# Gabriel-SGama/Semantic-SuperPoint

Hardware: AMD Instinct MI355X
Metric: image-pairs/sec at 240x320 bs32 (pair training step) (higher is better)
Workload: dtype f32

## Files before the change

include/ssp_hip.h:

```cpp
#ifndef SSP_HIP_H
#define SSP_HIP_H

#include <stddef.h>
#include <stdint.h>

#ifdef __cplusplus
extern "C" {
#endif

typedef struct ssp_handle ssp_handle;

enum { SSP_ARCH_GAUSS2 = 0, SSP_ARCH_GAUSS2_SSMALL = 1 };
enum { SSP_NREP = 32 };

typedef struct {
  int arch;
  int n_classes;
  int max_batch;
  int height;
  int width;
  int n_match;
  int n_non;
  int dense_loss;
} ssp_config;
// ... 98 lines not shown
                      void* workspace_dev, size_t workspace_bytes, void* stream);

int ssp_op_conv_bf16(const void* in_dev, const float* w_oihw_dev, const float* bias_dev, void* out_dev, int n, int h, int w,
                     int cin, int cout, int ksize, int in_mode, const float* in_scale_dev, const float* in_shift_dev,
                     double* stats_dev, int transpose_flip, int in_f32, int out_f32, void* pool_out_dev,
                     const float* pool_gamma_dev, void* workspace_dev, size_t workspace_bytes, void* stream);

int ssp_op_conv_wgrad_bf16(const void* x_dev, const void* dy_dev, float* dw_oihw_dev, int n, int h, int w, int cin, int cout,
                           int ksize, int in_mode, const float* in_scale_dev, const float* in_shift_dev, int dy_f32,
                           void* workspace_dev, size_t workspace_bytes, void* stream);

int ssp_op_bn_bwd_bf16(const void* y_dev, const void* dout_dev, const float* gamma_dev, const float* stats4_dev, void* dy_dev,
                       float* dgamma_dev, float* dbeta_dev, float* dbias_dev, double* sums_dev, int n, int h, int w, int c, int cs,
                       int relu, int pool, void* stream);

int ssp_op_labels(const float* labels2d_dev, const float* mask2d_dev, float* target_dev, float* cellmask_dev, int b,
                  int h, int w, void* stream);

int ssp_op_detector_loss(const float* semi_nhwc_dev, int cs, const float* labels2d_dev, const float* mask2d_dev, int b, int h,
                         int w, void* scratch_dev, size_t scratch_bytes, float* loss_dev, float* dsemi_nhwc_dev, void* stream);

int ssp_op_sem_loss(const float* sout_nhwc_dev, int cs, const int64_t* labels_dev, int b, int h, int w, int n_classes, int algo,
                    void* scratch_dev, size_t scratch_bytes, float* loss_dev, float* dsout_nhwc_dev, void* stream);

int ssp_op_sem_predict(const float* sout_nhwc_dev, int cs, const int64_t* labels_dev, int b, int h, int w, int n_classes,
                       uint8_t* pred_dev, int64_t* confusion_dev, void* stream);
int ssp_sem_predict(ssp_handle* h, int slot, const int64_t* labels_dev, uint8_t* pred_dev, int64_t* confusion_dev, void* stream);

int ssp_op_warp_image(const float* img_dev, const float* inv_h_dev, float* out_dev, int b, int h, int w, int nearest,
                      void* stream);
// ... 276 lines not shown
```

semantic-superpoint_amd/csrc/bn_kernels.hip.h:

```cpp
#pragma once
#include <hip/hip_runtime.h>
#include <stdint.h>

#include "conv_mfma.hip.h"

namespace sspk {

template <typename T>
__device__ __forceinline__ float4 ld4(const T* p) {
  if constexpr (sizeof(T) == 4) {
    return *reinterpret_cast<const float4*>(p);
  } else {
    const u32x2 v = *reinterpret_cast<const u32x2*>(p);
    return make_float4(bf16_lo(v[0]), bf16_hi(v[0]), bf16_lo(v[1]), bf16_hi(v[1]));
  }
}
template <typename T>
__device__ __forceinline__ void st4(T* p, float4 v) {
  if constexpr (sizeof(T) == 4) {
    *reinterpret_cast<float4*>(p) = v;
  } else {
    u32x2 o;
    o[0] = pack_bf16(v.x, v.y);
    o[1] = pack_bf16(v.z, v.w);
// ... 639 lines not shown
#pragma unroll
    for (int t = 0; t < 9; ++t) red[tid * 10 + t] = wacc[i >> 1][t][i & 1];
    __syncthreads();
    if (tid < 160) {
      const int qq = tid / 10, t = tid - qq * 10;
      if (t < 9) {
        float sum = 0.f;
#pragma unroll
        for (int r = 0; r < 16; ++r) sum += red[(r * 16 + qq) * 10 + t];
        facc_add(dw + (qq * 4 + i) * 9 + t, sum);
      }
    }
  }
}

template <typename T = float>
__device__ __forceinline__ void bn_bwd_sums_body(const BnBwdArgs& a0, const BnBwdArgs& a1, int nviews, float* __restrict__ dgamma,
                                                 float* __restrict__ dbeta) {
  const int t = blockIdx.x * blockDim.x + threadIdx.x;
  if ((t >> 5) >= ((a0.C + 7) & ~7)) return;
  const int c = min(t >> 5, a0.C - 1), r = t & 31;
  const bool writer = r == 0 && (t >> 5) < a0.C;
  for (int v = 0; v < nviews; ++v) {
    const BnBwdArgs& a = v ? a1 : a0;
    const int C = a.C;
    double s1, s2;
    replica_sums(a.sums, C, c, r, s1, s2);
    if (a.pool_fix && a.gamma[c] == 0.f) {
      double part = 0.0;
      if (a.beta[c] > 0.f) {
// ... 197 lines not shown
```

semantic-superpoint_amd/csrc/ssp.hip:

```cpp
#include "../../include/ssp_hip.h"

#include <hip/hip_runtime.h>

#include <cmath>
#include <cstdarg>
#include <cstdio>
#include <cstdlib>
#include <algorithm>
#include <cstring>
#include <string>
#include <vector>

#include "bn_kernels.hip.h"
#include "conv_mfma.hip.h"
#include "conv1x1_group.hip.h"
#include "conv_wino.hip.h"
#include "conv_wino_pipe.hip.h"
#include "conv_wino_p2.hip.h"
#include "conv_wino4.hip.h"
#include "wgrad_wino4.hip.h"
#include "wgrad_wino_fused.hip.h"
#include "conv_bf16.hip.h"
#include "conv_bf16_ws.hip.h"
#include "wgrad_bf16.hip.h"
// ... 136 lines not shown
  float *wpk_fwd, *wpk_bwd, *wpk_heads_bwd;
  float* partial;
  size_t partial_floats;
  size_t partial_used = 0;
  struct WredBQueue* rq_bf16 = nullptr;
  WredJobs rjobs{};
  bool bsums_fused[16] = {};
  bool sums_lazy[16] = {};
  bool fin_pending[16] = {};
  double fin_count[16] = {};
  bool apply_fused[16] = {};
  bool bf16_fuse_apply = true;
  StepAccum* accum;
  float* dots;
  bool desc_gather = true;
  int32_t *csr_off = nullptr, *csr_match = nullptr;
  float* csr_weight = nullptr;
  float* g_rows = nullptr;
  float* dense_coef;
  int sout_cs;
  int conv_algo;
  bool pk_w4_fwd[16] = {}, pk_w4_bwd[16] = {};
  float *wpk_g1_fwd[16] = {}, *wpk_g1_bwd[16] = {};
  bool pk_g1[16] = {};
  float* g1_partial = nullptr;
  TailJobs tail = {};
  int g1_partial_slabs = 0;
  int packed_algo = -1;
  bool packed_bwd = false;
  struct GraphEntry { std::vector<unsigned char> key; hipGraphExec_t exec; };
// ... 915 lines not shown
  const BnBwdArgs& a1 = a[nviews - 1];
  const int nq = (a0.C + 3) / 4, rows = 256 / nq;
  const long npix = (long)a0.N * (POOL ? a0.H / 2 : a0.H) * (POOL ? a0.W / 2 : a0.W);
  int nb = cdiv(npix, rows);
  if (nb > 1024) nb = 1024;
  if (!sums_done)
    hipLaunchKernelGGL((bn_bwd_kernel<RELU, POOL, false, T>), dim3(nb, nviews), dim3(256), 0, st, a0, a1, a0, a1);
  hipLaunchKernelGGL(bn_bwd_sums_kernel<T>, dim3(cdiv(a0.C * 32, 256)), dim3(256), 0, st, a0, a1, nviews, dgamma, dbeta);
  if (!skip_apply)
    hipLaunchKernelGGL((bn_bwd_kernel<RELU, POOL, true, T>), dim3(nb, nviews), dim3(256), 0, st, a0, a1, a0, a1);
  HIPCHK(hipGetLastError());
  return 0;
}

template <typename K>
static int l0_resident_grid(K kern, const ssp_handle* h, int nviews, long rows, int W) {
  static int per_cu = 0, per_cu_w = 0;
  if (per_cu_w != W) { per_cu = 0; per_cu_w = W; }
  if (per_cu == 0 && (hipOccupancyMaxActiveBlocksPerMultiprocessor(&per_cu, kern, 256, l0_lds_bytes(W)) != hipSuccess || per_cu < 1)) {
    (void)hipGetLastError();
    per_cu = -1;
  }
  if (per_cu < 1) return l0_grid(rows);
  const long g = std::max(1L, (long)per_cu * (h ? h->n_cu : 256) / std::max(1, nviews));
  return (int)std::min(rows, g);
}

#include "bf16_host.hip.h"

static int flush_wgrad_reduce_bf16(ssp_handle* h, hipStream_t st) { return h->rq_bf16 != nullptr ? h->rq_bf16->flush(st) : 0; }

static int ensure_aux_stream(ssp_handle* h);
static bool desc_gather_env();

struct DetHostRegion { float* lo; size_t n; long long* shadow; const ssp_handle* owner; };
static std::vector<DetHostRegion> g_det_regions;
static int g_det_mode = -1;
static int g_det_device = -1;
static bool det_mode() {
  if (g_det_mode < 0) { const char* e = getenv("SSP_DETERMINISTIC"); g_det_mode = (e != nullptr && atoi(e) != 0) ? 1 : 0; }
  return g_det_mode == 1;
}
static int det_upload() {
  DetRegion tab[DET_MAX_REGIONS];
  int n = 0;
  for (const DetHostRegion& r : g_det_regions) {
    if (n == DET_MAX_REGIONS) return fail(-3, "deterministic mode: more than %d fp32 scatter targets are bound in this process", DET_MAX_REGIONS);
    tab[n].lo = r.lo; tab[n].hi = r.lo + r.n; tab[n].shadow = r.shadow; ++n;
// ... 109 lines not shown
int ssp_create(const ssp_config* cfg, ssp_handle** out) {
  if (!cfg || !out) return fail(-1, "null argument");
  if (cfg->arch != SSP_ARCH_GAUSS2 && cfg->arch != SSP_ARCH_GAUSS2_SSMALL) return fail(-1, "unknown arch %d", cfg->arch);
  if (cfg->height % 8 || cfg->width % 8 || cfg->height <= 0 || cfg->width <= 0)
    return fail(-1, "height/width must be positive multiples of 8 (got %dx%d)", cfg->height, cfg->width);
  if (cfg->width > L0_MAX_W) return fail(-1, "width must be <= %d (row images of the first-layer kernels)", L0_MAX_W);
  if (cfg->max_batch < 1 || cfg->max_batch > 1024) return fail(-1, "max_batch must be in 1..1024");
  if (cfg->arch == SSP_ARCH_GAUSS2_SSMALL && cfg->n_classes > 192) return fail(-1, "n_classes must be <= 192");
  ssp_handle* h = new ssp_handle();
  h->cfg = *cfg;
  if (h->cfg.n_classes <= 0) h->cfg.n_classes = 133;
  if (h->cfg.n_match <= 0) h->cfg.n_match = 1000;
  if (h->cfg.n_non <= 0) h->cfg.n_non = 100;
  h->conv_algo = g_default_conv_algo;
  h->desc_gather = desc_gather_env();
  h->rq_bf16 = new WredBQueue();
  AlgoScope algo(h);
  build_layers(h);
  h->bound = false;
  h->n_cu = device_cu_count();
  h->ws_bytes = carve(h, nullptr);
  h->prof_family = 0; h->ev_used = 0; h->prof_flops = h->prof_bytes = h->prof_exec_flops = 0; h->prof_launches = 0;
  *out = h;
  return 0;
}

void ssp_destroy(ssp_handle* h) {
  if (!h) return;
  det_release(h);
  delete h->rq_bf16;
// ... 481 lines not shown
  if (pack_forked) {
    CHK(ensure_aux_stream(h));
    CHK(pack_fork.fork(st, h->aux_stream, h->ev_pack_fork, h->ev_pack_join));
    CHK(pack_all(h, for_backward, SS.n, N, H, W, h->aux_stream));
  } else {
    CHK(pack_all(h, for_backward, SS.n, N, H, W, st));
  }
  {
    const LayerDesc& d = h->L[0];
    Slot &S0 = *SS.s[0], &S1 = *SS.s[SS.n - 1];
    if (bf16_path())
      hipLaunchKernelGGL(conv0_direct_kernel<uint16_t>, dim3(l0_resident_grid(conv0_direct_kernel<uint16_t>, h, SS.n, (long)N * H, W), SS.n), dim3(256), l0_lds_bytes(W), st, S0.x, S1.x, P(h, d.w_off),
                         P(h, d.b_off), reinterpret_cast<uint16_t*>(S0.Y[0]), reinterpret_cast<uint16_t*>(S1.Y[0]),
                         train ? S0.bn[0].stats : nullptr, train ? S1.bn[0].stats : nullptr, N, H, W);
    else
    hipLaunchKernelGGL(conv0_direct_kernel<float>, dim3(l0_resident_grid(conv0_direct_kernel<float>, h, SS.n, (long)N * H, W), SS.n), dim3(256), l0_lds_bytes(W), st, S0.x, S1.x, P(h, d.w_off),
                       P(h, d.b_off), S0.Y[0], S1.Y[0], train ? S0.bn[0].stats : nullptr, train ? S1.bn[0].stats : nullptr,
                       N, H, W);
    HIPCHK(hipGetLastError());
    if (train && bn_lazy_env() && !bf16_path()) { h->fin_pending[0] = true; h->fin_count[0] = (double)N * H * W; }
    else CHK(bn_finalize(h, SS.s, SS.n, 0, (double)N * H * W, train, st));
  }
  CHK(pack_fork.join());
  for (int l = 1; l < 8; ++l) {
    int lh, lw; layer_res(l, H, W, lh, lw);
    CHK(conv_layer_fwd(h, SS, l, l - 1, N, lh, lw, layer_in_mode(l), train, st));
  }
  const int Hc = H / 8, Wc = W / 8;
  auto pointwise = [&](const int* layers, int n) -> int {
    bool grouped = true;
    for (int i = 0; i < n; ++i) grouped = grouped && h->pk_g1[layers[i]];
    if (!grouped) {
      BnDeferred fin;
// ... 63 lines not shown
    v.dy_cs = dy_cs; v.dy_co = dy_co; v.count = (double)N * H * W;
    v.k12 = S.bn[l].k12;
    have_pool = have_pool && v.apool != nullptr;
  }
  const bool fused = h->bsums_fused[l];
  h->bsums_fused[l] = false;
  if (fused) h->tap_route[l] |= TAP_BSUMS_FUSED;
  h->apply_fused[l] = false;
  const bool raw_pool = pool_after && l < 8 && SS.s[0]->pool_raw[l];
  if ((fused || raw_pool) && pool_after)
    for (int k = 0; k < SS.n; ++k) a[k].pool_fix = 1;
  const BnBwdArgs &a0 = a[0], &a1 = a[SS.n - 1];
  float *dg = Gd(h, d.g_off), *db = Gd(h, d.be_off);
  if (l == 0) {
    const int nb1 = l0_resident_grid(bn_bwd_reduce_l0_kernel<float>, h, SS.n, (long)N * H, W);
    const int nb2 = l0_resident_grid(bn_bwd_apply_l0_kernel<float>, h, SS.n, (long)N * H, W);
    if (!fused)
      hipLaunchKernelGGL(bn_bwd_reduce_l0_kernel<float>, dim3(nb1, SS.n), dim3(256), l0_lds_bytes(W), st, a0, a1, P(h, d.w_off), P(h, d.b_off));
    hipLaunchKernelGGL(bn_bwd_sums_kernel<float>, dim3(cdiv(64 * 32, 256)), dim3(256), 0, st, a0, a1, SS.n, dg, db);
    hipLaunchKernelGGL(bn_bwd_apply_l0_kernel<float>, dim3(nb2, SS.n), dim3(256), l0_lds_bytes(W), st, a0, a1, P(h, d.w_off), P(h, d.b_off),
                       Gd(h, d.w_off));
    h->tap_route[0] |= TAP_WG_L0 << TAP_WG_SHIFT;
  } else if (relu && pool_after && have_pool && d.cout % 4 == 0 && d_cs == d.cout && d_co == 0) {
    const long npix = (long)N * (H / 2) * (W / 2);
    const int rows = 256 / (d.cout / 4);
    const int nb = std::max(1, std::min(cdiv(npix, rows), 1024));
    if (!fused && !SS.s[0]->pool_raw[l]) hipLaunchKernelGGL(bn_bwd_reduce_pool_kernel, dim3(nb, SS.n), dim3(256), 0, st, a0, a1, P(h, d.be_off));
    else if (!fused) {
      BnBwdArgs r[2] = {a[0], a[SS.n - 1]};
      for (int k = 0; k < 2; ++k) {
        r[k].y = r[k].apool; r[k].y_cs = d.cout; r[k].y_co = 0; r[k].H = H / 2; r[k].W = W / 2;
      }
      hipLaunchKernelGGL((bn_bwd_kernel<true, false, false>), dim3(nb, SS.n), dim3(256), 0, st, r[0], r[1], r[0], r[1]);
    }
    hipLaunchKernelGGL(bn_bwd_sums_kernel<float>, dim3(cdiv(d.cout * 32, 256)), dim3(256), 0, st, a0, a1, SS.n, dg, db);
    const bool defer = l >= 1 && l < 8 && layer_in_mode(l) == 1 && dy_cs == d.cout && dy_co == 0 && SS.s[0]->y_cs[l] == d.cout &&
// ... 938 lines not shown
}

int ssp_pair_step_phase(ssp_handle* h, const ssp_pair_inputs* in, float* scalars_dev, int phase, void* stream) {
  return pair_step_impl(h, in, scalars_dev, phase, (hipStream_t)stream);
}

size_t ssp_grad_early_offset(const ssp_handle* h) { return h ? h->L[EARLY_SPLIT_LAYER].w_off : 0; }

int ssp_pair_step_graph(ssp_handle* h, const ssp_pair_inputs* in, float* scalars_dev, int phase, int sample_indices,
                        void* stream) {
  if (!h || !h->bound) return fail(-1, "handle not bound");
  if (!in || !scalars_dev) return fail(-1, "null argument");
  hipStream_t st = (hipStream_t)stream;
  if (st == nullptr) return fail(-1, "ssp_pair_step_graph needs a non-default stream (stream capture)");
  if (h->tap_arena != nullptr) return fail(-1, "ssp_pair_step_graph: backward taps are on (ssp_debug_backward_taps); they need the eager step");
  std::vector<unsigned char> key(sizeof(ssp_pair_inputs) + sizeof(void*) + 5 * sizeof(int));
  {
    ssp_pair_inputs k;
    memcpy(&k, in, sizeof(k));
    k.seed = 0;
    memcpy(key.data(), &k, sizeof(k));
    memcpy(key.data() + sizeof(k), &scalars_dev, sizeof(void*));
    const int extra[5] = {phase, sample_indices, h->conv_algo, bf16_fuse_apply_env() ? 1 : 0,
                          h->desc_gather ? 1 : 0};
    memcpy(key.data() + sizeof(k) + sizeof(void*), extra, sizeof(extra));
  }
  hipGraphExec_t exec = nullptr;
  for (auto& g : h->graphs)
    if (g.key == key) { exec = g.exec; break; }
  if (exec == nullptr) {
    if (h->prof_family != 0) return fail(-1, "ssp_pair_step_graph: disable ssp_profile_enable before capturing");
    if (h->graphs.size() >= 16) {
      (void)hipGraphExecDestroy(h->graphs.front().exec);
      h->graphs.erase(h->graphs.begin());
    }
    hipGraph_t graph = nullptr;
    HIPCHK(hipStreamBeginCapture(st, hipStreamCaptureModeThreadLocal));
    int rc = 0;
    if (sample_indices && phase != 2) {
// ... 41 lines not shown
    if (workspace_bytes >= img) {
      hipStream_t st = (hipStream_t)stream;
      float* wpk = reinterpret_cast<float*>(workspace_dev);
      G1PackJobs G;
      G.n = 0;
      int nb = 0;
      g1_add_pack(G, nb, w_oihw_dev, wpk, transpose_flip ? cin : cout, transpose_flip ? cout : cin, transpose_flip ? 1 : 0);
      hipLaunchKernelGGL(pack_g1_kernel, dim3(nb), dim3(256), 0, st, G);
      HIPCHK(hipGetLastError());
      G1Layer y;
      y.in[0] = in_dev; y.in_cs = cin; y.in_co = 0; y.out[0] = out_dev; y.out_cs = cout; y.out_co = 0; y.wpk = wpk; y.bias = bias_dev;
      y.scale[0] = in_scale_dev; y.shift[0] = in_shift_dev; y.stats[0] = stats_dev; y.K = cin; y.N = cout;
      return launch_g1(&y, 1, 1, (long)n * hh * w, in_mode, device_cu_count(), st);
    }
  }
  const bool wino = wino_ok(ksize, cin) && in_mode != 2;
  const int nchunks = cdiv(cin, CK), ncob = cdiv(cout, NB);
  const size_t need = (size_t)ncob * nchunks * pk_taps(ksize) * CK * NB * sizeof(float);
  if (workspace_bytes < need) return fail(-4, "ssp_op_conv workspace too small (%zu < %zu)", workspace_bytes, need);
  if (bf16_path() && ksize == 3 && cin % CK == 0 && in_mode != 2)
    return fail(-3, "ssp_op_conv: conv algorithm 12 has no fp32 3x3 kernel for Cin %% 16 == 0 (use ssp_op_conv_bf16 or another algorithm)");
  hipStream_t st = (hipStream_t)stream;
  float* wpk = reinterpret_cast<float*>(workspace_dev);
  const bool w4 = wino && ksize == 3 && w4_eligible(nullptr, 1, n, hh, w, cin, cout);
  if (!transpose_flip) CHK(launch_pack(w_oihw_dev, wpk, cout, cin, ksize, 0, wino, st, w4));
  else CHK(launch_pack(w_oihw_dev, wpk, cin, cout, ksize, 1, wino, st, w4));
  ConvCall c;
  c.in = in_dev; c.in_cs = cin; c.in_co = 0; c.cin = cin; c.wpk = wpk; c.bias = bias_dev; c.out = out_dev; c.out_cs = cout;
  c.out_co = 0; c.cout = cout; c.in_scale = in_scale_dev; c.in_shift = in_shift_dev; c.stats = stats_dev; c.N = n;
  c.H = hh; c.W = w; c.ks = ksize; c.in_mode = in_mode; c.nchunks = nchunks; c.ncob = ncob; c.wino = wino;
// ... 1257 lines not shown
  HIPCHK(hipMemsetAsync(sums_dev, 0, 2 * (size_t)c * NREP * sizeof(double), st));
  BnBwdArgs a;
  a.y = y_dev; a.dout = dout_dev; a.dy = dy_dev; a.scale = stats4_dev; a.shift = stats4_dev + c; a.mean = stats4_dev + 2 * c;
  a.invstd = stats4_dev + 3 * c; a.gamma = gamma_dev; a.sums = sums_dev; a.dbias = dbias_dev; a.N = n; a.H = hh; a.W = w;
  a.C = c; a.y_cs = cs; a.y_co = 0; a.d_cs = cs; a.d_co = 0; a.dy_cs = cs; a.dy_co = 0; a.count = (double)n * hh * w;
  float* k12 = nullptr;
  HIPCHK(hipMallocAsync((void**)&k12, 2 * c * sizeof(float), st));
  a.k12 = k12; a.x = nullptr; a.apool = nullptr; a.beta = nullptr; a.pool_fix = 0;
  if (relu && pool) CHK((launch_bn_bwd<true, true>(&a, 1, dgamma_dev, dbeta_dev, st)));
  else if (relu) CHK((launch_bn_bwd<true, false>(&a, 1, dgamma_dev, dbeta_dev, st)));
  else CHK((launch_bn_bwd<false, false>(&a, 1, dgamma_dev, dbeta_dev, st)));
  HIPCHK(hipFreeAsync(k12, st));
  return 0;
}

int ssp_op_bn_bwd_bf16(const void* y_dev, const void* dout_dev, const float* gamma_dev, const float* stats4_dev, void* dy_dev,
                       float* dgamma_dev, float* dbeta_dev, float* dbias_dev, double* sums_dev, int n, int hh, int w, int c, int cs,
                       int relu, int pool, void* stream) {
  if (cs < c || (cs & 3)) return fail(-1, "ssp_op_bn_bwd_bf16: the channel stride must be a multiple of 4 and >= C");
  if (!relu) return fail(-3, "ssp_op_bn_bwd_bf16: only the ReLU layers run on bf16 tensors");
  hipStream_t st = (hipStream_t)stream;
  HIPCHK(hipMemsetAsync(sums_dev, 0, 2 * (size_t)c * NREP * sizeof(double), st));
  BnBwdArgs a;
  a.y = reinterpret_cast<const float*>(y_dev); a.dout = reinterpret_cast<const float*>(dout_dev); a.dy = reinterpret_cast<float*>(dy_dev);
  a.scale = stats4_dev; a.shift = stats4_dev + c; a.mean = stats4_dev + 2 * c;
  a.invstd = stats4_dev + 3 * c; a.gamma = gamma_dev; a.sums = sums_dev; a.dbias = dbias_dev; a.N = n; a.H = hh; a.W = w;
  a.C = c; a.y_cs = cs; a.y_co = 0; a.d_cs = cs; a.d_co = 0; a.dy_cs = cs; a.dy_co = 0; a.count = (double)n * hh * w;
  float* k12 = nullptr;
  HIPCHK(hipMallocAsync((void**)&k12, 2 * c * sizeof(float), st));
  a.k12 = k12; a.x = nullptr; a.apool = nullptr; a.beta = nullptr; a.pool_fix = 0;
// ... 295 lines not shown
```

semantic-superpoint_amd/lib.py:

```python
import ctypes as C
import math
import os
from collections import OrderedDict

import numpy as np
import torch

from . import hipbuild as _build

ARCHS = {"SuperPointNet_gauss2": 0, "SuperPointNet_gauss2_ssmall": 1}
SCALAR_NAMES = ["loss", "loss_det", "loss_det_warp", "loss_desc", "loss_sem", "loss_sem_warp", "positive_dist",
                "negative_dist", "eta_det", "eta_desc", "eta_sem"]
N_SCALARS = 16
NREP = 32
SAMPLER_MAX_MATCHES = 8192
PROF = {"none": 0, "conv3x3_fwd": 1, "conv3x3_dgrad": 2, "conv3x3_wgrad": 3, "conv_big_fwd": 4, "conv3x3_all": 5,
        "conv3x3_every": 6}
PROF_KERNELS = ["conv_wino4_kernel", "conv_wino_pipe_kernel", "conv_wino_p2_kernel", "wgrad_wino_kernel", "wgrad_wino4_kernel",
                "other", "conv_bf16_kernel", "wgrad_bf16_kernel"]


class SspConfig(C.Structure):
    _fields_ = [("arch", C.c_int), ("n_classes", C.c_int), ("max_batch", C.c_int), ("height", C.c_int),
                ("width", C.c_int), ("n_match", C.c_int), ("n_non", C.c_int), ("dense_loss", C.c_int)]
# ... 71 lines not shown
                ("nms_dist", C.c_int32), ("border_remove", C.c_int32), ("top_k", C.c_int32), ("subpixel", C.c_int32)]


_lib = None

EXPORTS = ["ssp_last_error", "ssp_create", "ssp_destroy", "ssp_param_count", "ssp_bn_channel_count",
           "ssp_bn_layer_count", "ssp_workspace_bytes", "ssp_bind", "ssp_forward", "ssp_backward", "ssp_zero_grad",
           "ssp_pair_step", "ssp_adam_step", "ssp_sample_indices", "ssp_profile_enable", "ssp_profile_read", "ssp_profile_read_executed",
           "ssp_op_conv", "ssp_op_conv_wgrad", "ssp_op_labels", "ssp_op_sparse_loss", "ssp_op_bn_bwd", "ssp_op_bn_bwd_strided",
           "ssp_debug_buffer", "ssp_debug_conv_knobs", "ssp_set_conv_algo", "ssp_op_warp_image", "ssp_op_erode", "ssp_op_warp_labels",
           "ssp_export_workspace_bytes", "ssp_export_max_points", "ssp_export_points", "ssp_op_homoadapt_views",
           "ssp_op_flatten_detection", "ssp_op_combine_heatmap", "ssp_op_heatmap_points", "ssp_op_soft_argmax_points", "ssp_detector_heatmap", "ssp_op_heatmap_nms", "ssp_op_dense_loss",
           "ssp_op_sample_homographies", "ssp_op_warp_labels_full", "ssp_op_sem_finalize", "ssp_adam_step_scaled",
           "ssp_pair_step_phase", "ssp_grad_early_offset", "ssp_pair_step_graph", "ssp_handle_set_conv_algo",
           "ssp_op_detector_loss", "ssp_debug_occupancy", "ssp_sample_indices_cell", "ssp_op_warp_labels_px",
           "ssp_op_warp_labels_full_px", "ssp_profile_read_kernel", "ssp_op_label_quantize", "ssp_profile_pause", "ssp_op_conv_bf16", "ssp_op_conv_wgrad_bf16", "ssp_op_bn_bwd_bf16", "ssp_build_id",
           "ssp_set_deterministic", "ssp_get_deterministic", "ssp_clock_probe", "ssp_op_sem_loss",
           "ssp_describe_workspace_bytes", "ssp_describe_points", "ssp_op_sample_descriptors", "ssp_match_workspace_bytes",
           "ssp_match_two_way", "ssp_debug_backward_taps", "ssp_debug_backward_tap_floats", "ssp_debug_backward_tap",
           "ssp_eval_repeatability", "ssp_eval_ransac_workspace_bytes", "ssp_eval_ransac",
           "ssp_op_photometric_draw", "ssp_op_photometric_apply",
           "ssp_shapes_workspace_bytes", "ssp_op_shapes_draw", "ssp_op_shapes_render", "ssp_op_warp_points_scatter",
           "ssp_op_sem_predict", "ssp_sem_predict",
           "ssp_track_workspace_bytes", "ssp_op_track_update", "ssp_op_track_select", "ssp_op_track_points",
           "ssp_op_point_classes", "ssp_point_classes", "ssp_filter_workspace_bytes", "ssp_op_filter_points",
           "ssp_match_two_way_classes",
           "ssp_det_eval_workspace_bytes", "ssp_op_det_tp_fp", "ssp_op_det_tp_fp_points", "ssp_det_pr_curve_workspace_bytes",
           "ssp_op_det_pr_curve", "ssp_op_sparse_loss_path",
           "ssp_eval_pixel_homographies", "ssp_eval_accumulate",
           "ssp_epi_ransac_workspace_bytes", "ssp_epi_ransac", "ssp_op_filter_matches",
           "ssp_pose_from_fundamental", "ssp_pose_chain",
# ... 108 lines not shown
        if os.environ.get("SSP_HIP_LIB") is None:
            raise
    lib.ssp_debug_buffer.argtypes = [vp, i, C.c_char_p, C.POINTER(vp), C.POINTER(C.c_size_t)]
    if hasattr(lib, "ssp_debug_backward_taps"):
        lib.ssp_debug_backward_taps.argtypes = [vp, vp, C.c_size_t, C.c_uint]
        lib.ssp_debug_backward_tap_floats.argtypes = [vp, C.c_uint]
        lib.ssp_debug_backward_tap_floats.restype = C.c_size_t
        lib.ssp_debug_backward_tap.argtypes = [vp, i, i, i, C.POINTER(C.c_size_t), C.POINTER(C.c_size_t), C.POINTER(C.c_uint)]
    lib.ssp_debug_conv_knobs.argtypes = [i, i]
    lib.ssp_debug_occupancy.argtypes = [i]
    lib.ssp_set_conv_algo.argtypes = [i]
    lib.ssp_op_warp_image.argtypes = [vp, vp, vp, i, i, i, i, vp]
    lib.ssp_op_erode.argtypes = [vp, vp, i, i, i, i, vp]
    lib.ssp_op_warp_labels.argtypes = [vp, vp, vp, i, i, i, vp]
    lib.ssp_op_bn_bwd.argtypes = [vp, vp, vp, vp, vp, vp, vp, vp, vp, i, i, i, i, i, i, vp]
    lib.ssp_op_bn_bwd_strided.argtypes = [vp, vp, vp, vp, vp, vp, vp, vp, vp, i, i, i, i, i, i, i, vp]
    lib.ssp_op_labels.argtypes = [vp, vp, vp, vp, i, i, i, vp]
    lib.ssp_op_sparse_loss.argtypes = [vp, vp, vp, vp, vp, i, i, i, i, i, i, i, C.c_float, C.c_float, vp, vp, vp, vp]
    try:
        lib.ssp_op_sparse_loss_path.argtypes = [vp, vp, vp, vp, vp, i, i, i, i, i, i, i, C.c_float, C.c_float, vp, vp, vp, i, vp, vp, vp, vp]
    except AttributeError:
        if os.environ.get("SSP_HIP_LIB") is None:
            raise
    ep = C.POINTER(SspExportParams)
    lib.ssp_export_workspace_bytes.argtypes = [ep]
    lib.ssp_export_workspace_bytes.restype = C.c_size_t
    lib.ssp_export_max_points.argtypes = [ep]
    lib.ssp_export_points.argtypes = [vp, ep, i] + [C.POINTER(vp)] * 7 + [vp]
    lib.ssp_op_homoadapt_views.argtypes = [vp, vp, vp, vp, i, i, i, vp]
    lib.ssp_op_flatten_detection.argtypes = [vp, vp, vp, i, i, i, vp]
# ... 961 lines not shown
    lib = load_library()
    _need_gpu(y_nhwc, "y")
    N, H, W, cs = y_nhwc.shape
    Cc = gamma.numel()
    dev = y_nhwc.device
    stats4 = torch.cat([scale, shift, mean, invstd]).contiguous()
    dy = torch.zeros_like(y_nhwc) if cs != Cc else torch.empty_like(y_nhwc)
    dg, db, dbias = (torch.zeros(Cc, dtype=torch.float32, device=dev) for _ in range(3))
    sums = torch.zeros(NREP * 2 * Cc, dtype=torch.float64, device=dev)
    with torch.cuda.device(dev):
        _check(lib.ssp_op_bn_bwd_strided(_ptr(y_nhwc), _ptr(dout_nhwc), _ptr(gamma), _ptr(stats4), _ptr(dy), _ptr(dg),
                                         _ptr(db), _ptr(dbias), _ptr(sums), N, H, W, Cc, cs, int(relu), int(pool), _stream()))
    return dy, dg, db, dbias


def op_bn_bwd_bf16(y_nhwc, dout_nhwc, gamma, scale, shift, mean, invstd, pool=False):
    lib = load_library()
    _need_gpu(y_nhwc, "y")
    if y_nhwc.dtype != torch.bfloat16 or dout_nhwc.dtype != torch.bfloat16:
        raise RuntimeError("y and dout must be bfloat16")
    N, H, W, cs = y_nhwc.shape
    Cc = gamma.numel()
    dev = y_nhwc.device
    stats4 = torch.cat([scale, shift, mean, invstd]).contiguous()
    dy = torch.zeros_like(y_nhwc)
    dg, db, dbias = (torch.zeros(Cc, dtype=torch.float32, device=dev) for _ in range(3))
    sums = torch.zeros(NREP * 2 * Cc, dtype=torch.float64, device=dev)
    with torch.cuda.device(dev):
        _check(lib.ssp_op_bn_bwd_bf16(_ptr(y_nhwc), _ptr(dout_nhwc), _ptr(gamma), _ptr(stats4), _ptr(dy), _ptr(dg), _ptr(db),
                                      _ptr(dbias), _ptr(sums), N, H, W, Cc, cs, 1, int(pool), _stream()))
# ... 1234 lines not shown
```

Before: 2439.

## Stream layer-0 BN-backward dout through an LDS ring with async buffer loads

Adds a layer-0 fused BN-backward/weight-gradient kernel that prefetches dout rows into a per-wave LDS ring buffer using buffer_load-to-LDS, with hand-written waitcnt and ds_read asm. Prefetches sit several slots ahead so global memory latency overlaps the recompute-and-accumulate math. It is enabled by default through an env toggle, with the old kernel kept as a fallback when LDS would exceed 64KB. It also adds a standalone l0 wgrad op, a conv0 fast path in the generic conv op, and a graph-cache key field. The extra LDS per block may lower occupancy.

```diff
diff --git a/include/ssp_hip.h b/include/ssp_hip.h
--- a/include/ssp_hip.h
+++ b/include/ssp_hip.h
@@ -136,6 +136,10 @@
                        float* dgamma_dev, float* dbeta_dev, float* dbias_dev, double* sums_dev, int n, int h, int w, int c, int cs,
                        int relu, int pool, void* stream);
 
+int ssp_op_l0_wgrad(const float* x_dev, const float* dout_dev, const float* w0_dev, const float* b0_dev, const float* gamma_dev,
+                    const float* stats4_dev, float* dw0_dev, float* dgamma_dev, float* dbeta_dev, double* sums_dev, int n, int h,
+                    int w, void* stream);
+
 int ssp_op_labels(const float* labels2d_dev, const float* mask2d_dev, float* target_dev, float* cellmask_dev, int b,
                   int h, int w, void* stream);
 
diff --git a/semantic-superpoint_amd/csrc/bn_kernels.hip.h b/semantic-superpoint_amd/csrc/bn_kernels.hip.h
--- a/semantic-superpoint_amd/csrc/bn_kernels.hip.h
+++ b/semantic-superpoint_amd/csrc/bn_kernels.hip.h
@@ -677,6 +677,134 @@
   }
 }
 
+constexpr int L0R_DP = 4;
+static inline size_t l0_ring_lds_bytes(int W) { return (size_t)4 * L0R_DP * 2048 + l0_lds_bytes(W) + 32 * sizeof(float); }
+__global__ __launch_bounds__(256) void bn_bwd_apply_l0_ring_kernel(const BnBwdArgs a0, const BnBwdArgs a1,
+                                                                   const float* __restrict__ w0, const float* __restrict__ b0,
+                                                                   float* __restrict__ dw) {
+  const BnBwdArgs& a = blockIdx.y ? a1 : a0;
+  const float* __restrict__ x = a.x;
+  extern __shared__ float l0_rows[];
+  float* const red = l0_rows;
+  float* const imgs = l0_rows + 4 * L0R_DP * 512;
+  static_assert(4 * L0R_DP * 512 >= 256 * 10, "the weight-gradient reduction runs in the ring's LDS");
+  const int tid = threadIdx.x;
+  const int q = tid & 15, pl = tid >> 4;
+  const int wave = tid >> 6, lane = tid & 63;
+  const int c0 = q * 4;
+  L0Conv cv;
+  cv.load(w0, b0, c0);
+  f32x2 sc2[2], sh2[2], is2[2], nm2[2], nk1[2], nk2[2], gs2[2];
+#pragma unroll
+  for (int h = 0; h < 2; ++h) {
+    const int c = c0 + 2 * h;
+    sc2[h] = f32x2{a.scale[c], a.scale[c + 1]}; sh2[h] = f32x2{a.shift[c], a.shift[c + 1]};
+    is2[h] = f32x2{a.invstd[c], a.invstd[c + 1]};
+    nm2[h] = f32x2{-a.mean[c] * a.invstd[c], -a.mean[c + 1] * a.invstd[c + 1]};
+    nk1[h] = f32x2{-a.k12[c], -a.k12[c + 1]};
+    nk2[h] = f32x2{-a.k12[64 + c], -a.k12[64 + c + 1]};
+    gs2[h] = f32x2{a.gamma[c] * a.invstd[c], a.gamma[c + 1] * a.invstd[c + 1]};
+  }
+  f32x2 wacc[2][9];
+#pragma unroll
+  for (int h = 0; h < 2; ++h)
+#pragma unroll
+    for (int t = 0; t < 9; ++t) wacc[h][t] = f32x2{0.f, 0.f};
+  const int rows = a.N * a.H, W = a.W;
+  const int K2 = (W + 31) >> 5;
+  typedef __attribute__((address_space(3))) void* ldsp;
+  float* const myring = l0_rows + wave * (L0R_DP * 512);
+  const float* const myslot = myring + lane * 4;
+  int f_row = blockIdx.x, f_kk = 0;
+  auto issue = [&](int slot) __attribute__((always_inline)) {
+    const bool live = f_row < rows;
+    const __amdgpu_buffer_rsrc_t rs = __builtin_amdgcn_make_buffer_rsrc(
+        const_cast<float*>(a.dout) + (size_t)(live ? f_row : 0) * W * 64, 0, live ? W * 256 : 0, 0x00020000);
+    const unsigned vo = (unsigned)(lane * 16 + (32 * f_kk + 4 * wave) * 256);
+    __builtin_amdgcn_raw_ptr_buffer_load_lds(rs, (ldsp)(myring + slot * 512), 16, vo, 0, 0, 0);
+    __builtin_amdgcn_raw_ptr_buffer_load_lds(rs, (ldsp)(myring + slot * 512 + 256), 16, vo + 16 * 256, 0, 0, 0);
+    if (++f_kk == K2) { f_kk = 0; f_row += gridDim.x; }
+  };
+  for (int i = tid; i < 2 * 3 * (W + 2) + 32; i += 256) imgs[i] = 0.f;
+  __syncthreads();
+#pragma unroll
+  for (int s = 0; s < L0R_DP; ++s) issue(s);
+  int slot = 0, par = 0;
+  const int Wp = W + 2;
+  for (int row = blockIdx.x; row < rows; row += gridDim.x, par ^= 1) {
+    const int oy = row % a.H;
+    const bool up = oy > 0, down = oy < a.H - 1;
+    const float* xr = x + (size_t)row * W;
+    float* const img = imgs + par * 3 * Wp;
+    l0_stage_rows(img, xr, up, down, W);
+    __syncthreads();
+    const unsigned img_a = (unsigned)(size_t)(ldsp)(img + pl);
+    for (int kk = 0; kk < K2; ++kk) {
+      f32x4 d4[2];
+      float xv[2][9];
+      const unsigned ring_a = (unsigned)(size_t)(ldsp)(myslot + slot * 512);
+      const unsigned r0 = img_a + (unsigned)kk * 128u, r1 = r0 + (unsigned)Wp * 4u, r2 = r1 + (unsigned)Wp * 4u;
+      asm volatile(
+          "s_waitcnt vmcnt(%24)\n\t"
+          "ds_read_b128 %0, %20\n\t"
+          "ds_read_b128 %1, %20 offset:1024\n\t"
+          "ds_read_b32 %2, %21\n\tds_read_b32 %3, %21 offset:4\n\tds_read_b32 %4, %21 offset:8\n\t"
+          "ds_read_b32 %5, %22\n\tds_read_b32 %6, %22 offset:4\n\tds_read_b32 %7, %22 offset:8\n\t"
+          "ds_read_b32 %8, %23\n\tds_read_b32 %9, %23 offset:4\n\tds_read_b32 %10, %23 offset:8\n\t"
+          "ds_read_b32 %11, %21 offset:64\n\tds_read_b32 %12, %21 offset:68\n\tds_read_b32 %13, %21 offset:72\n\t"
+          "ds_read_b32 %14, %22 offset:64\n\tds_read_b32 %15, %22 offset:68\n\tds_read_b32 %16, %22 offset:72\n\t"
+          "ds_read_b32 %17, %23 offset:64\n\tds_read_b32 %18, %23 offset:68\n\tds_read_b32 %19, %23 offset:72\n\t"
+          "s_waitcnt lgkmcnt(0)"
+          : "=&v"(d4[0]), "=&v"(d4[1]), "=&v"(xv[0][0]), "=&v"(xv[0][1]), "=&v"(xv[0][2]), "=&v"(xv[0][3]), "=&v"(xv[0][4]),
+            "=&v"(xv[0][5]), "=&v"(xv[0][6]), "=&v"(xv[0][7]), "=&v"(xv[0][8]), "=&v"(xv[1][0]), "=&v"(xv[1][1]), "=&v"(xv[1][2]),
+            "=&v"(xv[1][3]), "=&v"(xv[1][4]), "=&v"(xv[1][5]), "=&v"(xv[1][6]), "=&v"(xv[1][7]), "=&v"(xv[1][8])
+          : "v"(ring_a), "v"(r0), "v"(r1), "v"(r2), "n"(2 * (L0R_DP - 1))
+          : "memory");
+      issue(slot);
+      slot = slot + 1 == L0R_DP ? 0 : slot + 1;
+      const bool ok[2] = {pl + 32 * kk < W, pl + 32 * kk + 16 < W};
+#pragma unroll
+      for (int j = 0; j < 2; ++j) {
+        const float dv[4] = {d4[j][0], d4[j][1], d4[j][2], d4[j][3]};
+        const float okf = ok[j] ? 1.f : 0.f;
+        L0Taps xt;
+        xt.set(xv[j]);
+#pragma unroll
+        for (int h = 0; h < 2; ++h) {
+          const f32x2 yv = cv.y2(h, xt);
+          const f32x2 z = pk_fma(yv, sc2[h], sh2[h]);
+          const f32x2 dz = {z[0] > 0.f ? dv[2 * h] : 0.f, z[1] > 0.f ? dv[2 * h + 1] : 0.f};
+          const f32x2 xh = pk_fma(yv, is2[h], nm2[h]);
+          const f32x2 g = pk_mul(pk_mul(gs2[h], f32x2{okf, okf}), pk_fma(xh, nk2[h], pk_add(dz, nk1[h])));
+#pragma unroll
+          for (int k = 0; k < 4; ++k) {
+            wacc[h][2 * k] = pk_fma_bcast<false>(xt.p[k], g, wacc[h][2 * k]);
+            wacc[h][2 * k + 1] = pk_fma_bcast<true>(xt.p[k], g, wacc[h][2 * k + 1]);
+          }
+          wacc[h][8] = pk_fma_bcast<false>(xt.p[4], g, wacc[h][8]);
+        }
+      }
+    }
+  }
+  asm volatile("s_waitcnt vmcnt(0)" : : : "memory");
+#pragma unroll
+  for (int i = 0; i < 4; ++i) {
+    __syncthreads();
+#pragma unroll
+    for (int t = 0; t < 9; ++t) red[tid * 10 + t] = wacc[i >> 1][t][i & 1];
+    __syncthreads();
+    if (tid < 160) {
+      const int qq = tid / 10, t = tid - qq * 10;
+      if (t < 9) {
+        float sum = 0.f;
+#pragma unroll
+        for (int r = 0; r < 16; ++r) sum += red[(r * 16 + qq) * 10 + t];
+        facc_add(dw + (qq * 4 + i) * 9 + t, sum);
+      }
+    }
+  }
+}
+
 template <typename T = float>
 __device__ __forceinline__ void bn_bwd_sums_body(const BnBwdArgs& a0, const BnBwdArgs& a1, int nviews, float* __restrict__ dgamma,
                                                  float* __restrict__ dbeta) {
diff --git a/semantic-superpoint_amd/csrc/ssp.hip b/semantic-superpoint_amd/csrc/ssp.hip
--- a/semantic-superpoint_amd/csrc/ssp.hip
+++ b/semantic-superpoint_amd/csrc/ssp.hip
@@ -174,6 +174,7 @@
   StepAccum* accum;
   float* dots;
   bool desc_gather = true;
+  bool l0_stream = true;
   int32_t *csr_off = nullptr, *csr_match = nullptr;
   float* csr_weight = nullptr;
   float* g_rows = nullptr;
@@ -1119,10 +1120,11 @@
 }
 
 template <typename K>
-static int l0_resident_grid(K kern, const ssp_handle* h, int nviews, long rows, int W) {
+static int l0_resident_grid(K kern, const ssp_handle* h, int nviews, long rows, int W, size_t lds_bytes = 0) {
   static int per_cu = 0, per_cu_w = 0;
-  if (per_cu_w != W) { per_cu = 0; per_cu_w = W; }
-  if (per_cu == 0 && (hipOccupancyMaxActiveBlocksPerMultiprocessor(&per_cu, kern, 256, l0_lds_bytes(W)) != hipSuccess || per_cu < 1)) {
+  static const void* per_cu_k = nullptr;
+  if (per_cu_w != W || per_cu_k != reinterpret_cast<const void*>(kern)) { per_cu = 0; per_cu_w = W; per_cu_k = reinterpret_cast<const void*>(kern); }
+  if (per_cu == 0 && (hipOccupancyMaxActiveBlocksPerMultiprocessor(&per_cu, kern, 256, lds_bytes ? lds_bytes : l0_lds_bytes(W)) != hipSuccess || per_cu < 1)) {
     (void)hipGetLastError();
     per_cu = -1;
   }
@@ -1137,6 +1139,32 @@
 
 static int ensure_aux_stream(ssp_handle* h);
 static bool desc_gather_env();
+static bool l0_stream_env() {
+  static const int v = getenv("SSP_L0_STREAM") ? atoi(getenv("SSP_L0_STREAM")) : 1;
+  return v != 0;
+}
+static int launch_apply_l0_f32(const ssp_handle* h, bool stream, int nviews, const BnBwdArgs& a0, const BnBwdArgs& a1, const float* w0,
+                               const float* b0, float* dw, hipStream_t st) {
+  const long rows = (long)a0.N * a0.H;
+  const int W = a0.W;
+  if (stream && l0_ring_lds_bytes(W) <= 64 * 1024) {
+    const size_t lds = l0_ring_lds_bytes(W);
+    hipLaunchKernelGGL(bn_bwd_apply_l0_ring_kernel, dim3(l0_resident_grid(bn_bwd_apply_l0_ring_kernel, h, nviews, rows, W, lds), nviews),
+                       dim3(256), lds, st, a0, a1, w0, b0, dw);
+  } else {
+    hipLaunchKernelGGL(bn_bwd_apply_l0_kernel<float>, dim3(l0_resident_grid(bn_bwd_apply_l0_kernel<float>, h, nviews, rows, W), nviews),
+                       dim3(256), l0_lds_bytes(W), st, a0, a1, w0, b0, dw);
+  }
+  HIPCHK(hipGetLastError());
+  return 0;
+}
+static int launch_conv0_f32(const ssp_handle* h, int nviews, const float* x0, const float* x1, const float* w, const float* bias,
+                            float* y0, float* y1, double* st0, double* st1, int N, int H, int W, hipStream_t st) {
+  hipLaunchKernelGGL(conv0_direct_kernel<float>, dim3(l0_resident_grid(conv0_direct_kernel<float>, h, nviews, (long)N * H, W), nviews),
+                     dim3(256), l0_lds_bytes(W), st, x0, x1, w, bias, y0, y1, st0, st1, N, H, W);
+  HIPCHK(hipGetLastError());
+  return 0;
+}
 
 struct DetHostRegion { float* lo; size_t n; long long* shadow; const ssp_handle* owner; };
 static std::vector<DetHostRegion> g_det_regions;
@@ -1276,6 +1304,7 @@
   if (h->cfg.n_non <= 0) h->cfg.n_non = 100;
   h->conv_algo = g_default_conv_algo;
   h->desc_gather = desc_gather_env();
+  h->l0_stream = l0_stream_env();
   h->rq_bf16 = new WredBQueue();
   AlgoScope algo(h);
   build_layers(h);
@@ -1787,9 +1816,8 @@
                          P(h, d.b_off), reinterpret_cast<uint16_t*>(S0.Y[0]), reinterpret_cast<uint16_t*>(S1.Y[0]),
                          train ? S0.bn[0].stats : nullptr, train ? S1.bn[0].stats : nullptr, N, H, W);
     else
-    hipLaunchKernelGGL(conv0_direct_kernel<float>, dim3(l0_resident_grid(conv0_direct_kernel<float>, h, SS.n, (long)N * H, W), SS.n), dim3(256), l0_lds_bytes(W), st, S0.x, S1.x, P(h, d.w_off),
-                       P(h, d.b_off), S0.Y[0], S1.Y[0], train ? S0.bn[0].stats : nullptr, train ? S1.bn[0].stats : nullptr,
-                       N, H, W);
+      CHK(launch_conv0_f32(h, SS.n, S0.x, S1.x, P(h, d.w_off), P(h, d.b_off), S0.Y[0], S1.Y[0], train ? S0.bn[0].stats : nullptr,
+                           train ? S1.bn[0].stats : nullptr, N, H, W, st));
     HIPCHK(hipGetLastError());
     if (train && bn_lazy_env() && !bf16_path()) { h->fin_pending[0] = true; h->fin_count[0] = (double)N * H * W; }
     else CHK(bn_finalize(h, SS.s, SS.n, 0, (double)N * H * W, train, st));
@@ -1883,12 +1911,10 @@
   float *dg = Gd(h, d.g_off), *db = Gd(h, d.be_off);
   if (l == 0) {
     const int nb1 = l0_resident_grid(bn_bwd_reduce_l0_kernel<float>, h, SS.n, (long)N * H, W);
-    const int nb2 = l0_resident_grid(bn_bwd_apply_l0_kernel<float>, h, SS.n, (long)N * H, W);
     if (!fused)
       hipLaunchKernelGGL(bn_bwd_reduce_l0_kernel<float>, dim3(nb1, SS.n), dim3(256), l0_lds_bytes(W), st, a0, a1, P(h, d.w_off), P(h, d.b_off));
     hipLaunchKernelGGL(bn_bwd_sums_kernel<float>, dim3(cdiv(64 * 32, 256)), dim3(256), 0, st, a0, a1, SS.n, dg, db);
-    hipLaunchKernelGGL(bn_bwd_apply_l0_kernel<float>, dim3(nb2, SS.n), dim3(256), l0_lds_bytes(W), st, a0, a1, P(h, d.w_off), P(h, d.b_off),
-                       Gd(h, d.w_off));
+    CHK(launch_apply_l0_f32(h, h->l0_stream, SS.n, a0, a1, P(h, d.w_off), P(h, d.b_off), Gd(h, d.w_off), st));
     h->tap_route[0] |= TAP_WG_L0 << TAP_WG_SHIFT;
   } else if (relu && pool_after && have_pool && d.cout % 4 == 0 && d_cs == d.cout && d_co == 0) {
     const long npix = (long)N * (H / 2) * (W / 2);
@@ -2857,15 +2883,15 @@
   hipStream_t st = (hipStream_t)stream;
   if (st == nullptr) return fail(-1, "ssp_pair_step_graph needs a non-default stream (stream capture)");
   if (h->tap_arena != nullptr) return fail(-1, "ssp_pair_step_graph: backward taps are on (ssp_debug_backward_taps); they need the eager step");
-  std::vector<unsigned char> key(sizeof(ssp_pair_inputs) + sizeof(void*) + 5 * sizeof(int));
+  std::vector<unsigned char> key(sizeof(ssp_pair_inputs) + sizeof(void*) + 6 * sizeof(int));
   {
     ssp_pair_inputs k;
     memcpy(&k, in, sizeof(k));
     k.seed = 0;
     memcpy(key.data(), &k, sizeof(k));
     memcpy(key.data() + sizeof(k), &scalars_dev, sizeof(void*));
-    const int extra[5] = {phase, sample_indices, h->conv_algo, bf16_fuse_apply_env() ? 1 : 0,
-                          h->desc_gather ? 1 : 0};
+    const int extra[6] = {phase, sample_indices, h->conv_algo, bf16_fuse_apply_env() ? 1 : 0,
+                          h->desc_gather ? 1 : 0, h->l0_stream ? 1 : 0};
     memcpy(key.data() + sizeof(k) + sizeof(void*), extra, sizeof(extra));
   }
   hipGraphExec_t exec = nullptr;
@@ -2937,6 +2963,9 @@
       return launch_g1(&y, 1, 1, (long)n * hh * w, in_mode, device_cu_count(), st);
     }
   }
+  if (cin == 1 && cout == 64 && ksize == 3 && in_mode == 0 && !transpose_flip && bias_dev != nullptr && w <= L0_MAX_W && !bf16_path())
+    return launch_conv0_f32(nullptr, 1, in_dev, in_dev, w_oihw_dev, bias_dev, out_dev, out_dev, stats_dev, stats_dev, n, hh, w,
+                            (hipStream_t)stream);
   const bool wino = wino_ok(ksize, cin) && in_mode != 2;
   const int nchunks = cdiv(cin, CK), ncob = cdiv(cout, NB);
   const size_t need = (size_t)ncob * nchunks * pk_taps(ksize) * CK * NB * sizeof(float);
@@ -4224,6 +4253,42 @@
   return 0;
 }
 
+int ssp_op_l0_wgrad(const float* x_dev, const float* dout_dev, const float* w0_dev, const float* b0_dev, const float* gamma_dev,
+                    const float* stats4_dev, float* dw0_dev, float* dgamma_dev, float* dbeta_dev, double* sums_dev, int n, int hh,
+                    int w, void* stream) {
+  if (n < 1 || hh < 1 || w < 1 || w > L0_MAX_W) return fail(-1, "ssp_op_l0_wgrad: bad shape %d x %d x %d", n, hh, w);
+  hipStream_t st = (hipStream_t)stream;
+  const int c = 64;
+  static const int det_tag = 0;
+  const ssp_handle* const det_owner = reinterpret_cast<const ssp_handle*>(&det_tag);
+  const bool det = det_mode();
+  if (det) {
+    CHK(det_register(det_owner, dw0_dev, (size_t)c * 9));
+    CHK(det_upload());
+  }
+  HIPCHK(hipMemsetAsync(sums_dev, 0, 2 * (size_t)c * NREP * sizeof(double), st));
+  BnBwdArgs a;
+  a.y = nullptr; a.dout = dout_dev; a.dy = nullptr; a.scale = stats4_dev; a.shift = stats4_dev + c; a.mean = stats4_dev + 2 * c;
+  a.invstd = stats4_dev + 3 * c; a.gamma = gamma_dev; a.sums = sums_dev; a.dbias = nullptr; a.N = n; a.H = hh; a.W = w;
+  a.C = c; a.y_cs = c; a.y_co = 0; a.d_cs = c; a.d_co = 0; a.dy_cs = c; a.dy_co = 0; a.count = (double)n * hh * w;
+  float* k12 = nullptr;
+  HIPCHK(hipMallocAsync((void**)&k12, 2 * c * sizeof(float), st));
+  a.k12 = k12; a.x = x_dev; a.apool = nullptr; a.beta = nullptr; a.pool_fix = 0;
+  const long rows = (long)n * hh;
+  hipLaunchKernelGGL(bn_bwd_reduce_l0_kernel<float>, dim3(l0_resident_grid(bn_bwd_reduce_l0_kernel<float>, nullptr, 1, rows, w)), dim3(256),
+                     l0_lds_bytes(w), st, a, a, w0_dev, b0_dev);
+  hipLaunchKernelGGL(bn_bwd_sums_kernel<float>, dim3(cdiv(c * 32, 256)), dim3(256), 0, st, a, a, 1, dgamma_dev, dbeta_dev);
+  hipError_t le = hipGetLastError();
+  if (le == hipSuccess && launch_apply_l0_f32(nullptr, l0_stream_env(), 1, a, a, w0_dev, b0_dev, dw0_dev, st) != 0) le = hipErrorLaunchFailure;
+  int rc = le == hipSuccess ? det_fold(dw0_dev, st) : fail(-2, "ssp_op_l0_wgrad: %s", hipGetErrorString(le));
+  if (hipFreeAsync(k12, st) != hipSuccess && rc == 0) rc = fail(-2, "ssp_op_l0_wgrad: hipFreeAsync");
+  if (det) {
+    if (hipStreamSynchronize(st) != hipSuccess && rc == 0) rc = fail(-2, "ssp_op_l0_wgrad: hipStreamSynchronize");
+    det_release(det_owner);
+  }
+  return rc;
+}
+
 int ssp_op_bn_bwd_bf16(const void* y_dev, const void* dout_dev, const float* gamma_dev, const float* stats4_dev, void* dy_dev,
                        float* dgamma_dev, float* dbeta_dev, float* dbias_dev, double* sums_dev, int n, int hh, int w, int c, int cs,
                        int relu, int pool, void* stream) {
diff --git a/semantic-superpoint_amd/lib.py b/semantic-superpoint_amd/lib.py
--- a/semantic-superpoint_amd/lib.py
+++ b/semantic-superpoint_amd/lib.py
@@ -109,7 +109,7 @@
            "ssp_op_sample_homographies", "ssp_op_warp_labels_full", "ssp_op_sem_finalize", "ssp_adam_step_scaled",
            "ssp_pair_step_phase", "ssp_grad_early_offset", "ssp_pair_step_graph", "ssp_handle_set_conv_algo",
            "ssp_op_detector_loss", "ssp_debug_occupancy", "ssp_sample_indices_cell", "ssp_op_warp_labels_px",
-           "ssp_op_warp_labels_full_px", "ssp_profile_read_kernel", "ssp_op_label_quantize", "ssp_profile_pause", "ssp_op_conv_bf16", "ssp_op_conv_wgrad_bf16", "ssp_op_bn_bwd_bf16", "ssp_build_id",
+           "ssp_op_warp_labels_full_px", "ssp_profile_read_kernel", "ssp_op_label_quantize", "ssp_profile_pause", "ssp_op_conv_bf16", "ssp_op_conv_wgrad_bf16", "ssp_op_bn_bwd_bf16", "ssp_op_l0_wgrad", "ssp_build_id",
            "ssp_set_deterministic", "ssp_get_deterministic", "ssp_clock_probe", "ssp_op_sem_loss",
            "ssp_describe_workspace_bytes", "ssp_describe_points", "ssp_op_sample_descriptors", "ssp_match_workspace_bytes",
            "ssp_match_two_way", "ssp_debug_backward_taps", "ssp_debug_backward_tap_floats", "ssp_debug_backward_tap",
@@ -248,6 +248,8 @@
     lib.ssp_op_erode.argtypes = [vp, vp, i, i, i, i, vp]
     lib.ssp_op_warp_labels.argtypes = [vp, vp, vp, i, i, i, vp]
     lib.ssp_op_bn_bwd.argtypes = [vp, vp, vp, vp, vp, vp, vp, vp, vp, i, i, i, i, i, i, vp]
+    if hasattr(lib, "ssp_op_l0_wgrad"):
+        lib.ssp_op_l0_wgrad.argtypes = [vp, vp, vp, vp, vp, vp, vp, vp, vp, vp, i, i, i, vp]
     lib.ssp_op_bn_bwd_strided.argtypes = [vp, vp, vp, vp, vp, vp, vp, vp, vp, i, i, i, i, i, i, i, vp]
     lib.ssp_op_labels.argtypes = [vp, vp, vp, vp, i, i, i, vp]
     lib.ssp_op_sparse_loss.argtypes = [vp, vp, vp, vp, vp, i, i, i, i, i, i, i, C.c_float, C.c_float, vp, vp, vp, vp]
@@ -1239,6 +1241,21 @@
     return dy, dg, db, dbias
 
 
+def op_l0_wgrad(x_nhw, dout_nhwc, w0, b0, gamma, scale, shift, mean, invstd):
+    lib = load_library()
+    _need_gpu(x_nhw, "x")
+    N, H, W = x_nhw.shape
+    dev = x_nhw.device
+    stats4 = torch.cat([scale, shift, mean, invstd]).contiguous()
+    dw = torch.zeros(64, 1, 3, 3, dtype=torch.float32, device=dev)
+    dg, db = (torch.zeros(64, dtype=torch.float32, device=dev) for _ in range(2))
+    sums = torch.zeros(NREP * 128, dtype=torch.float64, device=dev)
+    with torch.cuda.device(dev):
+        _check(lib.ssp_op_l0_wgrad(_ptr(x_nhw), _ptr(dout_nhwc), _ptr(w0), _ptr(b0), _ptr(gamma), _ptr(stats4), _ptr(dw), _ptr(dg),
+                                   _ptr(db), _ptr(sums), N, H, W, _stream()))
+    return dw, dg, db
+
+
 def op_bn_bwd_bf16(y_nhwc, dout_nhwc, gamma, scale, shift, mean, invstd, pool=False):
     lib = load_library()
     _need_gpu(y_nhwc, "y")
```

After: 2436. About the same (-0.1%).
